# joesound212985/Deepfake-Detection-using-CLIP-Based-SigLIP-2-Vision-Transformers

Hardware: AMD Instinct MI355X
Metric: images/sec (train fwd+bwd) SigLIP-2-so400m@384 bf16 (higher is better)
Workload: dtype bf16; 1 GPU; so400m-patch14-384 encoder+pool-head train fwd+bwd, 384x384, per-GPU batch 128, seeded random weights; global_batch=128, parallelism=dp1

## Files before the change

deepfake-detection-using-clip-based-siglip-2-vision-transformers_amd/csrc/attention.hip:

```cpp
#include <stdlib.h>

#include "attention.hip.h"

namespace sgl {

template <int DP>
struct AttnCfg {
  static constexpr int KS = DP / 16;
  static constexpr int DT = (DP + 31) / 32;
  static constexpr int CPR = DP / 8;
  static constexpr int RSTR = DP * 2 + 16;
  static constexpr int TSTR = 192;
  static constexpr int DSTR = 208;
  static constexpr int DIMG = (32 * (DSTR / 16) + 63) / 64 * 1024;
  static constexpr int RIMG = (32 * (RSTR / 16) + 63) / 64 * 1024;
  static constexpr int SMEM_FWD = 2 * (64 * RSTR + 64 * TSTR);
  static constexpr int SMEM_KV = 3 * (2 * DIMG + 32 * 8);
  static constexpr int SMEM_Q = 3 * (DIMG + RIMG);
};

__device__ __forceinline__ u32x4 a_ldg(__amdgpu_buffer_rsrc_t r, uint32_t off) {
  return __builtin_amdgcn_raw_buffer_load_b128(r, off, 0, 0);
}
template <typename T>
// ... 317 lines not shown
        for (int r = 0; r < 16; ++r) o[dt][r] *= alpha;
    }
    lo_x8<T> pb[4];
    pb[0] = pack8<T>(s0, 0);
    pb[1] = pack8<T>(s0, 8);
    pb[2] = pack8<T>(s1, 0);
    pb[3] = pack8<T>(s1, 8);
#pragma unroll
    for (int dt = 0; dt < C::DT; ++dt)
#pragma unroll
      for (int kk = 0; kk < 4; ++kk) o[dt] = MFMA32(lds_trfrag<T>(vb, C::TSTR, kk, dt * 32, lane), pb[kk], o[dt]);
  }
  const float l = l_run + __shfl_xor(l_run, 32, 64);
  const float inv = 1.0f / l;
  const int q = q0 + qi;
  if (q < N) {
    T* orow = out + (size_t)(sb.row0 + q) * ((size_t)H * dh) + hd * dh;
#pragma unroll
    for (int dt = 0; dt < C::DT; ++dt)
#pragma unroll
      for (int g4 = 0; g4 < 4; ++g4) {
        const int d = dt * 32 + 8 * g4 + 4 * hh;
        if (d < dh) {
          lo_x4<T> v4;
#pragma unroll
          for (int r = 0; r < 4; ++r) v4[r] = (T)(o[dt][4 * g4 + r] * inv);
          *reinterpret_cast<lo_x4<T>*>(orow + d) = v4;
        }
      }
    if (hh == 0) lse[(size_t)hd * Ttot + sb.row0 + q] = m_run * scale + __logf(l);
  }
}

template <typename T, int DP, bool TOK>
__global__ __launch_bounds__(256, 2) void attn_bwd_kv_kernel(const T* __restrict__ Q, const T* __restrict__ K,
                                                             const T* __restrict__ V, const T* __restrict__ dO,
                                                             const float* __restrict__ aux, T* __restrict__ dqkv,
                                                             int B, int H, int N, int dh, int ld, float c, float scale) {
  using C = AttnCfg<DP>;
  constexpr int QT = 32;
  constexpr int SC = C::DSTR / 16;
  constexpr int NIS = (QT * SC + 63) / 64;
  constexpr int IMG = NIS * 1024;
  constexpr int STAGE = 2 * IMG + QT * 8;
  constexpr int NSLOT = 2 * NIS + 1;
  static_assert(NSLOT <= 16 && NSLOT > 12, "four DMA slots per wave (three for the last wave)");
  extern __shared__ __attribute__((aligned(16))) char smem[];
  const int t = threadIdx.x, lane = t & 63;
  const int w = __builtin_amdgcn_readfirstlane(t >> 6);
  int bh, xb;
  if (!head_block((N + 127) / 128, B * H, bh, xb)) return;
  const int b = bh / H, hd = bh - b * H;
  const int D = H * dh;
  const int key0 = xb * 128 + w * 32;
  HeadSrc src = head_src(TOK ? ld : 0, b, hd, H, N, dh, DP);
  if constexpr (!TOK) {
    src.rowbytes = (uint32_t)DP * 2u;
    src.nc = (uint32_t)DP / 8u;
  }
  const __amdgpu_buffer_rsrc_t rk = make_rsrc(K + src.base, src.bytes);
  const __amdgpu_buffer_rsrc_t rv = make_rsrc(V + src.base, src.bytes);
  const T* dOb = dO + (size_t)b * N * D + hd * dh;
  const u32x4 dq_ = att_desc(Q + src.base, src.bytes);
  const u32x4 ddo = att_desc(dOb, (uint32_t)(((size_t)(N - 1) * D + dh) * 2));
  const u32x4 dax = att_desc(aux + (size_t)bh * N * 2, (uint32_t)((size_t)N * 8));
  const uint32_t lds0 = (uint32_t)(size_t)((SGL_LDS char*)smem);
// ... 324 lines not shown
#pragma unroll
          for (int r = 0; r < 4; ++r) a[r] = (T)dq[dt][4 * g4 + r];
          *reinterpret_cast<lo_x4<T>*>(qrow + d) = a;
        }
      }
  }
}

bool attn_shape_ok(int dtype, int B, int H, int N, int dh, int DP, int ld, AttnPass pass) {
  const bool probs = pass == ATTN_PROBS, strict = dtype == DT_F32, f32m = dtype == DT_F32_MFMA;
  const bool lo = !strict && !f32m;
  if (probs && (B < 1 || H < 1 || N < 1 || dh < 1 || dh > DP)) return false;
  if (strict) {
    if (dh > 128) return false;
  } else {
    if (dh % 8) return false;
    if (f32m && (dh > 96 || DP < dh || DP % 4)) return false;
    if (lo && (DP != ((dh + 15) / 16) * 16 || !attn_dp_ok(DP))) return false;
    if (ld < 0 || (ld > 0 && (ld % (lo ? 8 : 4) || ld < H * dh))) return false;
  }
  if (f32m && N <= 0) return false;
  if (lo) {
    if ((size_t)N * (ld > 0 ? ld : DP) * 2 >= (1ull << 31)) return false;
    if (!probs && (size_t)N * H * dh * 2 >= (1ull << 31)) return false;
  }
  if (strict && !probs && attn_ref_lds(N, pass == ATTN_BWD ? 2 : 1, pass == ATTN_BWD ? 2 : 1) > 160 * 1024) return false;
  if (probs) {
    const size_t wgs = strict ? (size_t)((N + 3) / 4) * ((N + 63) / 64) : (size_t)((N + 127) / 128) * ((N + 127) / 128);
    if (wgs * (size_t)B * (size_t)H >= (1ull << 31)) return false;
  }
  return true;
}

hipError_t attn_fwd(const void* q, const void* k, const void* v, int dtype, void* out, float* lse, int B, int H, int N,
                    int dh, int DP, int ld, hipStream_t s) {
  if (B * H == 0 || N == 0) return hipSuccess;
  if (!attn_shape_ok(dtype, B, H, N, dh, DP, ld, ATTN_FWD)) return hipErrorInvalidValue;
  if (dtype == DT_F32)
    return attn_ref_fwd((const float*)q, (const float*)k, (const float*)v, (float*)out, lse, B, H, N, dh, DP, ld, s);
  if (dtype == DT_F32_MFMA)
    return attn_f32_fwd((const float*)q, (const float*)k, (const float*)v, (float*)out, lse, B, H, N, dh, DP, ld, s);
  if (!attn_aligned16(q, k, v)) return hipErrorInvalidValue;
  const AttnScales sc = attn_scales(dh);
  return dispatch_attn(dtype, DP, [&](auto tag) {
    using T = typename decltype(tag)::type;
    constexpr int DPV = decltype(tag)::dp;
    return with_bool(ld > 0, [&](auto tok) {
      hipLaunchKernelGGL((attn_fwd_kernel<T, DPV, tok.value>), head_grid((N + 127) / 128, B * H), dim3(256),
                         AttnCfg<DPV>::SMEM_FWD, s, (const T*)q, (const T*)k, (const T*)v, (T*)out, lse, B, H, N, dh,
                         tok.value ? ld : 0, sc.c, sc.scale);
      return hipGetLastError();
    });
  });
}

bool attn_varlen_shape_ok(int dtype, int S, int T, int max_n, int H, int dh, int DP) {
  if (S < 1 || T < 1 || max_n < 1 || H < 1 || dh < 1 || dh > DP) return false;
  if (!attn_shape_ok(dtype, 1, H, max_n, dh, DP, 0, ATTN_FWD)) return false;
  const int rows = dtype == DT_F32 ? 4 : 128;
  return seg_grid_ok(S, H, (max_n + rows - 1) / rows);
}

hipError_t attn_fwd_varlen(const void* q, const void* k, const void* v, int dtype, void* out, float* lse, const int* cu,
                           int S, int T, int max_n, int H, int dh, int DP, hipStream_t s) {
  if (!attn_varlen_shape_ok(dtype, S, T, max_n, H, dh, DP)) return hipErrorInvalidValue;
  if (dtype == DT_F32)
    return attn_ref_fwd_varlen((const float*)q, (const float*)k, (const float*)v, (float*)out, lse, cu, S, T, max_n, H, dh,
                               DP, s);
  if (dtype == DT_F32_MFMA)
    return attn_f32_fwd_varlen((const float*)q, (const float*)k, (const float*)v, (float*)out, lse, cu, S, T, max_n, H, dh,
                               DP, s);
  if (!attn_aligned16(q, k, v)) return hipErrorInvalidValue;
  const AttnScales sc = attn_scales(dh);
  return dispatch_attn(dtype, DP, [&](auto tag) {
    using T16 = typename decltype(tag)::type;
    constexpr int DPV = decltype(tag)::dp;
    hipLaunchKernelGGL((attn_fwd_varlen_kernel<T16, DPV>), seg_grid((max_n + 127) / 128, S * H), dim3(256),
                       AttnCfg<DPV>::SMEM_FWD, s, (const T16*)q, (const T16*)k, (const T16*)v, (T16*)out, lse, cu, S, T,
                       max_n, H, dh, sc.c, sc.scale);
// ... 36 lines not shown
```

deepfake-detection-using-clip-based-siglip-2-vision-transformers_amd/csrc/attention.hip.h:

```cpp
#pragma once
#include <math.h>

#include <type_traits>

#include "common.hip.h"
#include "kernels.h"

namespace sgl {

constexpr float kLog2e = SGL_LOG2E;
struct AttnScales {
  float scale, c;
};
static inline AttnScales attn_scales(int dh) {
  const float scale = 1.0f / sqrtf((float)dh);
  return {scale, scale * kLog2e};
}

__host__ __device__ constexpr int ctile_row(int i, int hh) { return 8 * (i >> 2) + 4 * hh + (i & 3); }

struct HeadSrc {
  uint32_t rowbytes, nc, bytes;
  size_t base;
};
// ... 27 lines not shown
  row0 = lo;
  n = min(hi - lo, max_n);
}
__device__ __forceinline__ bool seg_block(const int* __restrict__ cu, int S, int T, int max_n, int H, int nb, int rows,
                                          SegBlock& sb) {
  const int pid = blockIdx.x, xcd = pid & 7, slot = pid >> 3;
  const int hq = slot / nb;
  const int sh = hq * 8 + xcd;
  if (sh >= S * H) return false;
  sb.xb = slot - hq * nb;
  sb.seg = sh / H;
  sb.hd = sh - sb.seg * H;
  seg_range(cu, sb.seg, T, max_n, sb.row0, sb.n);
  return sb.xb * rows < sb.n;
}
static inline dim3 seg_grid(int nb, int SH) { return dim3((unsigned)(8 * ((SH + 7) / 8) * nb)); }
static inline bool seg_grid_ok(int S, int H, int nb) { return (size_t)8 * (((size_t)S * H + 7) / 8) * (size_t)nb < (1ull << 31); }

constexpr int kAttnDP[] = {16, 32, 48, 64, 80, 96};
constexpr int kAttnNDP = sizeof(kAttnDP) / sizeof(kAttnDP[0]);
constexpr bool attn_dp_ok(int DP) {
  for (int i = 0; i < kAttnNDP; ++i)
    if (kAttnDP[i] == DP) return true;
  return false;
}
constexpr size_t attn_ref_lds(int N, int nvec, int nrow) { return (size_t)4 * (nvec * N + 128 * nrow) * sizeof(float); }

enum AttnPass : int { ATTN_FWD, ATTN_BWD, ATTN_PROBS };
bool attn_shape_ok(int dtype, int B, int H, int N, int dh, int DP, int ld, AttnPass pass);
static inline bool attn_aligned16(const void* a, const void* b, const void* c = nullptr) {
  return ((((uintptr_t)a) | ((uintptr_t)b) | ((uintptr_t)c)) & 15) == 0;
}

template <typename T, int DP>
struct AttnTag {
  using type = T;
  static constexpr int dp = DP;
};
template <typename T, int I = 0, typename F>
hipError_t dispatch_attn_dp(int DP, F&& f) {
  if constexpr (I == kAttnNDP) {
    return hipErrorInvalidValue;
  } else {
    if (DP == kAttnDP[I]) return f(AttnTag<T, kAttnDP[I]>{});
    return dispatch_attn_dp<T, I + 1>(DP, f);
  }
}
template <typename F>
hipError_t dispatch_attn(int dtype, int DP, F&& f) {
  return dtype == DT_F16 ? dispatch_attn_dp<f16>(DP, f) : dispatch_attn_dp<bf16>(DP, f);
}
template <typename F>
auto with_bool(bool flag, F&& f) {
  return flag ? f(std::true_type{}) : f(std::false_type{});
}

hipError_t attn_f32_fwd(const float* q, const float* k, const float* v, float* out, float* lse, int B, int H, int N, int dh,
                        int DP, int ld, hipStream_t s);
hipError_t attn_f32_bwd(const float* q, const float* k, const float* v, const float* out, const float* dout,
                        const float* lse, float* dqkv, float* delta, int B, int H, int N, int dh, int DP, int ld,
                        hipStream_t s);
hipError_t attn_ref_fwd(const float* q, const float* k, const float* v, float* out, float* lse, int B, int H, int N, int dh,
                        int DP, int ld, hipStream_t s);
hipError_t attn_ref_bwd(const float* q, const float* k, const float* v, const float* out, const float* dout,
                        const float* lse, float* dqkv, float* delta, int B, int H, int N, int dh, int DP, int ld,
                        hipStream_t s);
// ... 7 lines not shown
```

deepfake-detection-using-clip-based-siglip-2-vision-transformers_amd/csrc/encoder.hip:

```cpp
#include <hip/hip_runtime.h>
#include <string.h>

#include <algorithm>
#include <new>
#include <vector>

#include "kernels.h"
#include "siglip_hip.h"

using namespace sgl;

namespace {

inline size_t align256(size_t x) { return (x + 255) & ~(size_t)255; }
inline char* at(void* base, size_t off) { return reinterpret_cast<char*>(base) + off; }
inline const char* at(const void* base, size_t off) { return reinterpret_cast<const char*>(base) + off; }
inline bool mfma16(int dt) { return dt == DT_BF16 || dt == DT_F16; }
inline int round_up(int x, int m) { return (x + m - 1) / m * m; }

struct Bump {
  size_t off = 0;
  size_t take(size_t bytes) {
    const size_t o = off;
    off += align256(bytes);
// ... 1378 lines not shown
  else if (dtype == DT_F16)
    CKV(gemm_nt_f16(A, lda, B, ldb, M, N, K, epi, out_dt, p, (hipStream_t)stream));
  else
    CKV(gemm_f32_generic((const float*)A, lda, 1, (const float*)B, ldb, 1, M, N, K, epi, out_dt, p,
                         (hipStream_t)stream));
  return SGL_OK;
}

int sgl_op_gemm_tn(int dtype, const void* A, int lda, const void* B, int ldb, int Mred, int N1, int N2, int splits,
                   float* out, int ldo, int accumulate, sgl_stream stream) {
  return sgl_op_gemm_tn_ws(dtype, A, lda, B, ldb, Mred, N1, N2, splits, out, ldo, accumulate, nullptr, 0, stream);
}

int sgl_op_gemm_tn_ws(int dtype, const void* A, int lda, const void* B, int ldb, int Mred, int N1, int N2, int splits,
                      float* out, int ldo, int accumulate, float* scratch, size_t scratch_bytes, sgl_stream stream) {
  EpiParams p;
  p.out = out; p.ldo = ldo; p.accumulate = accumulate;
  if (dtype == DT_BF16)
    CKV(gemm_tn_bf16(A, lda, B, ldb, Mred, N1, N2, splits, p, (hipStream_t)stream, scratch, scratch_bytes));
  else if (dtype == DT_F16)
    CKV(gemm_tn_f16(A, lda, B, ldb, Mred, N1, N2, splits, p, (hipStream_t)stream, scratch, scratch_bytes));
  else
    CKV(gemm_f32_generic((const float*)A, 1, lda, (const float*)B, 1, ldb, N1, N2, Mred, EPI_F32, DT_F32, p,
                         (hipStream_t)stream));
  return SGL_OK;
}

int sgl_op_attn_fwd(int dtype, const void* q, const void* k, const void* v, void* out, float* lse, int B, int H, int N,
                    int head_dim, int head_dim_pad, int ld_qkv, sgl_stream stream) {
  CKV(attn_fwd(q, k, v, dtype, out, lse, B, H, N, head_dim, head_dim_pad, ld_qkv, (hipStream_t)stream));
  return SGL_OK;
}

int sgl_op_attn_bwd(int dtype, const void* q, const void* k, const void* v, const void* out, const void* dout,
                    const float* lse, void* dqkv, float* delta_scratch, int B, int H, int N, int head_dim,
                    int head_dim_pad, int ld_qkv, sgl_stream stream) {
  CKV(attn_bwd(q, k, v, out, dout, lse, dtype, dqkv, delta_scratch, B, H, N, head_dim, head_dim_pad, ld_qkv, (hipStream_t)stream));
  return SGL_OK;
}

int sgl_op_attn_probs(int dtype, const void* q, const void* k, const float* lse, float* out, int B, int H, int N,
                      int head_dim, int head_dim_pad, int mode, sgl_stream stream) {
  if (!q || !k || !lse || !out) return SGL_ERR_NULL;
  if (B < 1 || H < 1 || N < 1 || head_dim < 1 || head_dim_pad < 1 || head_dim > head_dim_pad) return SGL_ERR_BAD_SHAPE;
  if (dtype != DT_F32 && dtype != DT_BF16 && dtype != DT_F32_MFMA && dtype != DT_F16) return SGL_ERR_UNSUPPORTED;
  if (mode != SGL_ATTN_PROBS_FULL && mode != SGL_ATTN_PROBS_HEAD_MEAN) return SGL_ERR_UNSUPPORTED;
  if (!attn_probs_shape_ok(dtype, B, H, N, head_dim, head_dim_pad)) return SGL_ERR_BAD_SHAPE;
  CKV(attn_probs(q, k, lse, out, dtype, B, H, N, head_dim, head_dim_pad, mode, (hipStream_t)stream));
  return SGL_OK;
}

int sgl_op_attn_grad_probs(int dtype, const void* q, const void* k, const void* v, const void* dout, const float* lse,
                           float* out, int B, int H, int N, int head_dim, int head_dim_pad, int kind, int mode,
                           sgl_stream stream) {
  if (!q || !k || !v || !dout || !lse || !out) return SGL_ERR_NULL;
  if (B < 1 || H < 1 || N < 1 || head_dim < 1 || head_dim_pad < 1 || head_dim > head_dim_pad) return SGL_ERR_BAD_SHAPE;
  if (dtype != DT_F32 && dtype != DT_BF16 && dtype != DT_F32_MFMA && dtype != DT_F16) return SGL_ERR_UNSUPPORTED;
  if (mode != SGL_ATTN_PROBS_FULL && mode != SGL_ATTN_PROBS_HEAD_MEAN) return SGL_ERR_UNSUPPORTED;
  if (kind != SGL_ATTN_GRAD_DP && kind != SGL_ATTN_GRAD_PDP && kind != SGL_ATTN_GRAD_RELEVANCE) return SGL_ERR_UNSUPPORTED;
  if (!attn_grad_probs_shape_ok(dtype, B, H, N, head_dim, head_dim_pad)) return SGL_ERR_BAD_SHAPE;
  CKV(attn_grad_probs(q, k, v, dout, lse, out, dtype, B, H, N, head_dim, head_dim_pad, kind, mode, (hipStream_t)stream));
  return SGL_OK;
}

int sgl_attention_probs(sgl_ctx* ctx, int B, int H, int W, const void* saved, size_t saved_bytes, int layer, int mode,
                        float* out, size_t out_bytes, sgl_stream stream) {
// ... 233 lines not shown
```

deepfake-detection-using-clip-based-siglip-2-vision-transformers_amd/csrc/kernels.h:

```cpp
#pragma once
#include <hip/hip_runtime.h>
#include <stddef.h>
#include <stdint.h>

#include "siglip_hip.h"

namespace sgl {

enum DType : int {
  DT_F32 = 0,
  DT_BF16 = 1,
  DT_F32_MFMA = 2,
  DT_F16 = 3,
};
static inline size_t dtype_size(int dt) { return (dt == DT_BF16 || dt == DT_F16) ? 2 : 4; }

template <auto Kernel>
hipError_t set_max_dynamic_lds_once(int bytes) {
  static bool done = false;
  if (done) return hipSuccess;
  const hipError_t e =
      hipFuncSetAttribute(reinterpret_cast<const void*>(Kernel), hipFuncAttributeMaxDynamicSharedMemorySize, bytes);
  done = e == hipSuccess;
  return e;
// ... 142 lines not shown
constexpr TnPlan tn_plan(int Mred, int N1, int N2, size_t ws_bytes, int tile = 0) {
  TnPlan best = {0, 0, 0};
  long best_cost = 0;
  for (int g = 0; g < 2; ++g) {
    const int bm = g ? 384 : 256, bn = g ? 192 : 256, area8 = g ? 9 : 8;
    if (tile != 0 && tile != bm) continue;
    const int tiles = ((N1 + bm - 1) / bm) * ((N2 + bn - 1) / bn);
    for (int sp = 1; sp == 1 || (tiles * sp <= 256 && Mred / sp >= 1024); ++sp) {
      if (sp > 1 && (size_t)sp * N1 * N2 * sizeof(float) > ws_bytes) break;
      const int m_per = ((Mred + sp - 1) / sp + 63) / 64 * 64;
      const long cost = (long)area8 * m_per;
      if (best.tile == 0 || cost < best_cost) {
        best = {bm, (Mred + m_per - 1) / m_per, m_per};
        best_cost = cost;
      }
    }
  }
  return best;
}
constexpr bool tn_plan_is(int Mred, int N1, int N2, size_t ws_bytes, int tile, int splits) {
  const TnPlan p = tn_plan(Mred, N1, N2, ws_bytes);
  return (tile == 0 || p.tile == tile) && p.splits == splits;
}
constexpr size_t kTnSlabBytes = (size_t)256 * 384 * 192 * 4;
static_assert(tn_plan_is(93312, 1152, 1152, kTnSlabBytes, 384, 14), "out_proj dW");
static_assert(tn_plan_is(93312, 3456, 1152, kTnSlabBytes, 384, 4), "QKV dW");
static_assert(tn_plan_is(93312, 4304, 1152, kTnSlabBytes, 256, 3), "fc1 dW");
static_assert(tn_plan_is(93312, 1152, 4304, kTnSlabBytes, 256, 3), "fc2 dW");
static_assert(tn_plan_is(4133, 520, 1152, kTnSlabBytes, 0, 4) && tn_plan(4133, 520, 1152, kTnSlabBytes).m_per == 1088, "digest case");
static_assert(tn_plan_is(2048, 512, 512, kTnSlabBytes, 256, 2) && tn_plan(2048, 512, 512, kTnSlabBytes).m_per == 1024, "digest case");

hipError_t attn_fwd(const void* q, const void* k, const void* v, int dtype, void* out, float* lse, int B, int H,
                    int N, int dh, int DP, int ld_qkv, hipStream_t s);
bool attn_varlen_shape_ok(int dtype, int S, int T, int max_n, int H, int dh, int DP);
hipError_t attn_fwd_varlen(const void* q, const void* k, const void* v, int dtype, void* out, float* lse, const int* cu,
                           int S, int T, int max_n, int H, int dh, int DP, hipStream_t s);
hipError_t attn_bwd(const void* q, const void* k, const void* v, const void* out, const void* dout,
                    const float* lse, int dtype, void* dqkv, float* delta, int B, int H, int N, int dh, int DP,
                    int ld_qkv, hipStream_t s);

bool attn_probs_shape_ok(int dtype, int B, int H, int N, int dh, int DP);
hipError_t attn_probs(const void* q, const void* k, const float* lse, float* out, int dtype, int B, int H, int N, int dh,
                      int DP, int mode, hipStream_t s);
hipError_t probs_head_mean(const float* probs, float* out, int B, int H, int N, hipStream_t s);

bool attn_grad_probs_shape_ok(int dtype, int B, int H, int N, int dh, int DP);
hipError_t attn_grad_probs(const void* q, const void* k, const void* v, const void* dout, const float* lse, float* out,
                           int dtype, int B, int H, int N, int dh, int DP, int kind, int mode, hipStream_t s);
hipError_t pool_attn_grad_probs(const void* V, int dtype, const float* probs, const float* dout ,
                                float* out, int B, int H, int N, int dh, int DP, int kind, int mode, hipStream_t s);

}
```

deepfake-detection-using-clip-based-siglip-2-vision-transformers_amd/lib.py:

```python
from __future__ import annotations

import ctypes as C
import os
import re

_HERE = os.path.dirname(os.path.abspath(__file__))
LIB_PATH = os.environ.get("SGL_LIB_PATH") or os.path.join(_HERE, "libsiglip_hip.so")
HEADER_PATH = os.path.join(os.path.dirname(_HERE), "include", "siglip_hip.h")

SGL_DTYPE_F32, SGL_DTYPE_BF16, SGL_DTYPE_BF16X3, SGL_DTYPE_F16, SGL_DTYPE_MXFP8 = 0, 1, 2, 3, 5
SGL_DTYPE_U8 = 6
SEG_EVAL_AUC_BINS = 4096
SEG_TERM_FOCAL, SEG_TERM_BOUNDARY, SEG_TERM_TV = 1, 2, 4
SGL_RECOMPUTE_NONE, SGL_RECOMPUTE_BLOCKS = 0, 1
ATTN_PROBS_FULL, ATTN_PROBS_HEAD_MEAN = 0, 1
ATTN_GRAD_DP, ATTN_GRAD_PDP, ATTN_GRAD_RELEVANCE = 0, 1, 2
EPI_STORE, EPI_BIAS_GELU, EPI_RES_F32, EPI_QKV, EPI_GELU_BWD, EPI_POS_F32, EPI_F32 = range(7)
STATUS = {0: "ok", -1: "bad shape", -2: "unsupported configuration", -3: "buffer too small", -4: "HIP error",
          -5: "null pointer"}

_fp = C.c_void_p


class SglConfig(C.Structure):
# ... 105 lines not shown
    _sig(lib, "sgl_query_sizes_ragged", i, [C.c_void_p, C.POINTER(C.c_int), i, psz])
    _sig(lib, "sgl_forward_ragged", i, [C.c_void_p, C.POINTER(SglWeights), _fp, _fp, C.POINTER(C.c_int), i, C.POINTER(_fp),
                                        _fp, _fp, _fp, sz, _fp])
    _sig(lib, "sgl_backward_begin_p", i, [C.c_void_p, C.POINTER(SglWeights), _fp, C.POINTER(SglGrads), i, i, i, _fp, _fp,
                                          _fp, _fp, _fp, sz, _fp, sz, _fp])
    _sig(lib, "sgl_backward_layer_p", i, [C.c_void_p, C.POINTER(SglWeights), _fp, C.POINTER(SglGrads), i, i, i, i, _fp,
                                          _fp, i, _fp, sz, _fp, sz, _fp])
    preq = C.POINTER(SglAttnGradReq)
    _sig(lib, "sgl_backward_begin_pa", i, [C.c_void_p, C.POINTER(SglWeights), _fp, C.POINTER(SglGrads), i, i, i, _fp, _fp,
                                           _fp, _fp, _fp, sz, _fp, sz, _fp, preq])
    _sig(lib, "sgl_backward_layer_pa", i, [C.c_void_p, C.POINTER(SglWeights), _fp, C.POINTER(SglGrads), i, i, i, i, _fp,
                                           _fp, i, _fp, sz, _fp, sz, _fp, preq])
    _sig(lib, "sgl_backward_begin", i, [C.c_void_p, C.POINTER(SglWeights), _fp, C.POINTER(SglGrads), i, i, i, _fp, _fp,
                                        _fp, _fp, _fp, sz, _fp, sz, _fp])
    _sig(lib, "sgl_backward_layer", i, [C.c_void_p, C.POINTER(SglWeights), _fp, C.POINTER(SglGrads), i, i, i, i, _fp,
                                        _fp, i, _fp, sz, _fp, sz, _fp])
    _sig(lib, "sgl_backward_embed", i, [C.c_void_p, C.POINTER(SglWeights), C.POINTER(SglGrads), i, i, i, i, _fp, sz,
                                        _fp, sz, _fp])
    _sig(lib, "sgl_query_input_grad_bytes", i, [C.c_void_p, i, i, i, psz])
    _sig(lib, "sgl_backward_embed_px", i, [C.c_void_p, C.POINTER(SglWeights), C.POINTER(SglGrads), i, i, i, i, _fp, i, _fp,
                                           sz, _fp, sz, _fp, sz, _fp])
    _sig(lib, "sgl_backward", i, [C.c_void_p, C.POINTER(SglWeights), _fp, C.POINTER(SglGrads), i, i, i, i, _fp,
                                  C.POINTER(_fp), _fp, _fp, i, i, _fp, sz, _fp, sz, _fp])
    _sig(lib, "sgl_op_layernorm_fwd", i, [_fp, _fp, _fp, _fp, i, _fp, _fp, i, i, f, _fp])
    _sig(lib, "sgl_op_layernorm_bwd", i, [_fp, i, _fp, _fp, _fp, _fp, _fp, _fp, _fp, i, _fp, _fp, _fp, sz, i, i, _fp])
    _sig(lib, "sgl_op_gemm_nt", i, [i, _fp, i, _fp, i, i, i, i, i, _fp, i, _fp, i, _fp, _fp, i, _fp, i, _fp, i, i, i,
                                    i, i, i, _fp])
    _sig(lib, "sgl_op_quantize_mxfp8", i, [_fp, i, i, i, i, i, _fp, _fp, _fp])
    _sig(lib, "sgl_op_layernorm_fwd_mx", i, [_fp, _fp, _fp, _fp, _fp, i, i, i, f, _fp])
    _sig(lib, "sgl_op_gemm_nt_mx", i, [_fp, _fp, _fp, _fp, i, i, i, i, _fp, i, _fp, _fp, _fp, i, i, i, i, i, i, _fp])
    _sig(lib, "sgl_op_gemm_tn", i, [i, _fp, i, _fp, i, i, i, i, i, _fp, i, i, _fp])
    _sig(lib, "sgl_op_gemm_tn_ws", i, [i, _fp, i, _fp, i, i, i, i, i, _fp, i, i, _fp, sz, _fp])
    _sig(lib, "sgl_op_attn_fwd", i, [i, _fp, _fp, _fp, _fp, _fp, i, i, i, i, i, i, _fp])
    _sig(lib, "sgl_op_attn_bwd", i, [i, _fp, _fp, _fp, _fp, _fp, _fp, _fp, _fp, i, i, i, i, i, i, _fp])
    _sig(lib, "sgl_op_attn_probs", i, [i, _fp, _fp, _fp, _fp, i, i, i, i, i, i, _fp])
    _sig(lib, "sgl_op_attn_grad_probs", i, [i, _fp, _fp, _fp, _fp, _fp, _fp, i, i, i, i, i, i, i, _fp])
    _sig(lib, "sgl_op_pool_attn_grad_probs", i, [i, _fp, _fp, _fp, _fp, i, i, i, i, i, i, i, _fp])
    _sig(lib, "sgl_attention_probs", i, [C.c_void_p, i, i, i, _fp, sz, i, i, _fp, sz, _fp])
    _sig(lib, "sgl_op_colsum", i, [i, _fp, i, i, i, _fp, i, _fp, sz, _fp])
    _sig(lib, "sgl_op_im2col", i, [_fp, i, _fp, i, i, i, i, i, i, _fp])
    _sig(lib, "sgl_op_col2im", i, [_fp, i, i, i, i, i, _fp, i, _fp])
    _sig(lib, "sgl_op_pos_resize", i, [_fp, i, _fp, i, i, i, _fp])
    _sig(lib, "sgl_op_pool_attn_fwd", i, [i, _fp, _fp, _fp, _fp, _fp, i, i, i, i, i, _fp])
    _sig(lib, "sgl_op_attn_fwd_varlen", i, [i, _fp, _fp, _fp, _fp, _fp, _fp, i, i, i, i, i, i, _fp])
    _sig(lib, "sgl_op_pool_attn_fwd_varlen", i, [i, _fp, _fp, _fp, _fp, _fp, _fp, i, i, i, i, i, i, _fp])
    _sig(lib, "sgl_op_seg_offsets", i, [C.POINTER(C.c_int), i, _fp, _fp])
    _sig(lib, "sgl_op_pool_attn_bwd", i, [i, _fp, _fp, _fp, _fp, _fp, _fp, _fp, i, i, i, i, i, _fp])
    _sig(lib, "sgl_op_pos_resize_bwd", i, [_fp, i, i, _fp, i, i, _fp])
    _sig(lib, "sgl_op_cast_pad", i, [_fp, i, i, i, _fp, i, i, i, i, _fp])
    _sig(lib, "sgl_op_cast_job", i, [C.POINTER(SglCastMat), i, C.POINTER(SglCastVec), i, i, _fp])
    _sig(lib, "sgl_op_split3", i, [_fp, i, i, i, _fp, i, i, i, _fp])
    _sig(lib, "sgl_op_batch_sum", i, [_fp, i, sz, _fp, i, _fp])
    _sig(lib, "sgl_op_vecmat", i, [_fp, _fp, i, i, _fp, sz, _fp, i, _fp])
    _sig(lib, "sgl_op_reduce_partials", i, [_fp, i, i, _fp, i, i, _fp])
    _sig(lib, "sgl_op_reduce_partials3", i, [_fp, i, i, _fp, _fp, _fp, i, i, i, i, _fp])
    _sig(lib, "sgl_op_reduce_splits", i, [_fp, i, sz, i, i, _fp, i, i, _fp])
    _sig(lib, "sgl_op_add_f32", i, [_fp, _fp, _fp, sz, _fp])
    _sig(lib, "sgl_op_cast_f32", i, [_fp, _fp, i, sz, _fp])
    i64 = C.c_int64
    _sig(lib, "sgl_adamw_plan", i64, [C.POINTER(C.c_uint64), i, C.POINTER(C.c_int32), i64])
    _sig(lib, "sgl_op_grad_norm", i, [_fp, _fp, i64, f, _fp, _fp, _fp])
    _sig(lib, "sgl_op_adamw", i, [_fp, _fp, i64, C.c_double, C.c_double, C.c_double, i, _fp, _fp])
    _sig(lib, "sgl_op_ema", i, [_fp, _fp, i64, C.c_double, _fp])
    _sig(lib, "sgl_adamw_bind_shadows", i, [C.c_void_p, C.POINTER(SglWeights), _fp, C.POINTER(SglAdamwTensor),
                                            C.POINTER(SglAdamwAux), i])
    _sig(lib, "sgl_op_grad_norm_scaled", i, [_fp, _fp, i64, f, f, _fp, _fp, _fp])
# ... 73 lines not shown
```

include/siglip_hip.h:

```cpp
#ifndef SIGLIP_HIP_H
#define SIGLIP_HIP_H
#include <stddef.h>
#include <stdint.h>

#ifdef __cplusplus
extern "C" {
#endif

typedef struct sgl_ctx sgl_ctx;
typedef void* sgl_stream;

enum { SGL_DTYPE_F32 = 0, SGL_DTYPE_BF16 = 1, SGL_DTYPE_BF16X3 = 2, SGL_DTYPE_F16 = 3, SGL_DTYPE_MXFP8 = 5 };
enum { SGL_DTYPE_U8 = 6 };

typedef enum {
  SGL_OK = 0,
  SGL_ERR_BAD_SHAPE = -1,
  SGL_ERR_UNSUPPORTED = -2,
  SGL_ERR_WORKSPACE = -3,
  SGL_ERR_HIP = -4,
  SGL_ERR_NULL = -5
} sgl_status;

typedef struct {
// ... 96 lines not shown
int sgl_backward_embed_px(sgl_ctx* ctx, const sgl_weights* w, const sgl_grads* g, int B, int H, int W,
                          int interpolate_pos, float* d_pixels, int channels_last, void* px_scratch,
                          size_t px_scratch_bytes, const void* saved, size_t saved_bytes, void* ws, size_t ws_bytes,
                          sgl_stream stream);
int sgl_backward(sgl_ctx* ctx, const sgl_weights* w, const void* shadow, const sgl_grads* g, int B, int H, int W,
                 int interpolate_pos, const float* hidden_states, const float* const* d_taps,
                 const float* d_last_hidden, const float* d_pooled, int first_trainable_block, int train_embeddings,
                 const void* saved, size_t saved_bytes, void* ws, size_t ws_bytes, sgl_stream stream);

int sgl_op_layernorm_fwd(const float* x, const float* gamma, const float* beta, void* y, int y_dtype, float* mean,
                         float* rstd, int M, int D, float eps, sgl_stream stream);
int sgl_op_layernorm_bwd(const void* dy, int dy_dtype, const float* x, const float* mean, const float* rstd,
                         const float* gamma, const float* dres, float* dx, void* dx_lp, int lp_dtype, float* dgamma,
                         float* dbeta, float* scratch, size_t scratch_bytes, int M, int D, sgl_stream stream);
enum { SGL_EPI_STORE = 0, SGL_EPI_BIAS_GELU = 1, SGL_EPI_RES_F32 = 2, SGL_EPI_QKV = 3, SGL_EPI_GELU_BWD = 4,
       SGL_EPI_POS_F32 = 5, SGL_EPI_F32 = 6 };
int sgl_op_gemm_nt(int dtype, const void* A, int lda, const void* B, int ldb, int M, int N, int K, int epi, void* out,
                   int ldo, void* out2, int ldo2, const float* bias, const float* res, int ldr, const void* aux,
                   int ldaux, const float* pos, int pos_rows, int tokens, int heads, int head_dim, int head_dim_pad,
                   int batch, sgl_stream stream);
int sgl_op_quantize_mxfp8(const void* x, int x_dtype, int ldx, int M, int K, int Kp, void* q, void* scales,
                          sgl_stream stream);
int sgl_op_layernorm_fwd_mx(const float* x, const float* gamma, const float* beta, void* q, void* scales, int M, int D,
                            int Kp, float eps, sgl_stream stream);
int sgl_op_gemm_nt_mx(const void* A, const void* As, const void* B, const void* Bs, int M, int N, int Kp, int epi,
                      void* out, int ldo, void* out_scales, const float* bias, const float* res, int ldr, int tokens,
                      int heads, int head_dim, int head_dim_pad, int batch, sgl_stream stream);
int sgl_op_gemm_tn(int dtype, const void* A, int lda, const void* B, int ldb, int Mred, int N1, int N2, int splits,
                   float* out, int ldo, int accumulate, sgl_stream stream);
int sgl_op_gemm_tn_ws(int dtype, const void* A, int lda, const void* B, int ldb, int Mred, int N1, int N2, int splits,
                      float* out, int ldo, int accumulate, float* scratch, size_t scratch_bytes, sgl_stream stream);
int sgl_op_attn_fwd(int dtype, const void* q, const void* k, const void* v, void* out, float* lse, int B, int H, int N,
                    int head_dim, int head_dim_pad, int ld_qkv, sgl_stream stream);
int sgl_op_attn_bwd(int dtype, const void* q, const void* k, const void* v, const void* out, const void* dout,
                    const float* lse, void* dqkv, float* delta_scratch, int B, int H, int N, int head_dim,
                    int head_dim_pad, int ld_qkv, sgl_stream stream);
enum { SGL_ATTN_PROBS_FULL = 0, SGL_ATTN_PROBS_HEAD_MEAN = 1 };
int sgl_op_attn_probs(int dtype, const void* q, const void* k, const float* lse, float* out, int B, int H, int N,
                      int head_dim, int head_dim_pad, int mode, sgl_stream stream);
int sgl_attention_probs(sgl_ctx* ctx, int B, int H, int W, const void* saved, size_t saved_bytes, int layer, int mode,
                        float* out, size_t out_bytes, sgl_stream stream);
enum { SGL_ATTN_GRAD_DP = 0, SGL_ATTN_GRAD_PDP = 1, SGL_ATTN_GRAD_RELEVANCE = 2 };
int sgl_op_attn_grad_probs(int dtype, const void* q, const void* k, const void* v, const void* dout, const float* lse,
                           float* out, int B, int H, int N, int head_dim, int head_dim_pad, int kind, int mode,
                           sgl_stream stream);
int sgl_op_pool_attn_grad_probs(int dtype, const void* V, const float* probs, const float* dout, float* out, int B, int H,
                                int N, int head_dim, int head_dim_pad, int kind, int mode, sgl_stream stream);
typedef struct {
  float* out;
  size_t out_bytes;
  int kind;
  int mode;
} sgl_attn_grad_req;
int sgl_backward_layer_pa(sgl_ctx* ctx, const sgl_weights* w, const void* shadow, const sgl_grads* g, int layer, int B,
                          int H, int W, const float* hs_in, const float* d_tap, int need_dx, const void* saved,
                          size_t saved_bytes, void* ws, size_t ws_bytes, sgl_stream stream,
                          const sgl_attn_grad_req* req);
int sgl_backward_begin_pa(sgl_ctx* ctx, const sgl_weights* w, const void* shadow, const sgl_grads* g, int B, int H, int W,
                          const float* hs_last, const float* d_last_hidden, const float* d_pooled,
                          const float* d_tap_last, const void* saved, size_t saved_bytes, void* ws, size_t ws_bytes,
                          sgl_stream stream, const sgl_attn_grad_req* req);
int sgl_op_colsum(int dtype, const void* in, int ld, int M, int N, float* out, int accumulate, float* scratch,
                  size_t scratch_bytes, sgl_stream stream);
int sgl_op_im2col(const float* pixels, int channels_last, void* out, int out_dtype, int B, int H, int W, int P, int Kp,
                  sgl_stream stream);
int sgl_op_col2im(const float* d_cols, int B, int H, int W, int P, int Kp, float* d_pixels, int channels_last,
// ... 162 lines not shown
```

Before: 447.3 images/sec.

## Add 64-row-per-wave attention forward kernel reusing K/V fragments across query blocks

```diff
diff --git a/deepfake-detection-using-clip-based-siglip-2-vision-transformers_amd/csrc/attention.hip b/deepfake-detection-using-clip-based-siglip-2-vision-transformers_amd/csrc/attention.hip
--- a/deepfake-detection-using-clip-based-siglip-2-vision-transformers_amd/csrc/attention.hip
+++ b/deepfake-detection-using-clip-based-siglip-2-vision-transformers_amd/csrc/attention.hip
@@ -373,6 +373,175 @@
   }
 }
 
+template <typename T, int DP>
+__global__ __launch_bounds__(256, 2) void attn_fwd64_kernel(const T* __restrict__ Q, const T* __restrict__ K,
+                                                            const T* __restrict__ V, T* __restrict__ out,
+                                                            float* __restrict__ lse, int B, int H, int N, int dh, float c,
+                                                            float scale) {
+  using C = AttnCfg<DP>;
+  constexpr int KT = 64, NB = 2;
+  constexpr int KBYTES = KT * C::RSTR, VBYTES = KT * C::TSTR, STAGE = KBYTES + VBYTES;
+  constexpr int SCK = C::RSTR / 16, SCV = C::TSTR / 16;
+  constexpr int NIK = KT * SCK / 64, NIV = KT * SCV / 64, NSLOT = NIK + NIV;
+  constexpr int NPW = (NSLOT + 3) / 4;
+  extern __shared__ __attribute__((aligned(16))) char smem[];
+  const int t = threadIdx.x, lane = t & 63;
+  const int w = __builtin_amdgcn_readfirstlane(t >> 6);
+  int bh, xb;
+  if (!head_block((N + 255) / 256, B * H, bh, xb)) return;
+  const int b = bh / H, hd = bh - b * H;
+  const int q0 = xb * 256 + w * 64;
+  HeadSrc src = head_src(0, b, hd, H, N, dh, DP);
+  src.rowbytes = (uint32_t)DP * 2u;
+  src.nc = (uint32_t)DP / 8u;
+  const __amdgpu_buffer_rsrc_t rq = make_rsrc(Q + src.base, src.bytes);
+  const u32x4 dk_ = att_desc(K + src.base, src.bytes);
+  const u32x4 dv_ = att_desc(V + src.base, src.bytes);
+  const uint32_t lds0 = (uint32_t)(size_t)((SGL_LDS char*)smem);
+
+  const int qi = lane & 31, hh = lane >> 5;
+  lo_x8<T> qf[NB][C::KS];
+#pragma unroll
+  for (int blk = 0; blk < NB; ++blk)
+#pragma unroll
+    for (int ks = 0; ks < C::KS; ++ks) {
+      const uint32_t ch = (uint32_t)(2 * ks + hh);
+      const int qr = q0 + 32 * blk + qi;
+      qf[blk][ks] = as_x8<T>(a_ldg(rq, (qr < N && ch < src.nc) ? (uint32_t)qr * src.rowbytes + ch * 16u : SGL_OOB));
+    }
+
+  uint32_t voff[NPW];
+#pragma unroll
+  for (int j = 0; j < NPW; ++j) {
+    const int sl = w + 4 * j;
+    voff[j] = (sl < NIK) ? att_chunk_off(sl * 64 + lane, KT, SCK, (int)src.nc, src.rowbytes)
+                         : att_chunk_off((sl - NIK) * 64 + lane, KT, SCV, (int)src.nc, src.rowbytes);
+  }
+  const uint32_t tile_adv = (uint32_t)KT * src.rowbytes;
+  auto issue = [&](int stage) {
+    const uint32_t sb = lds0 + (uint32_t)(stage * STAGE);
+#pragma unroll
+    for (int j = 0; j < NPW; ++j) {
+      const int sl = w + 4 * j;
+      if (sl < NSLOT) att_dma16(sl < NIK ? dk_ : dv_, sb + (uint32_t)sl * 1024u, voff[j]);
+      voff[j] += tile_adv;
+    }
+  };
+
+  float m_run[NB], l_run[NB];
+  f32x16 o[NB][C::DT];
+#pragma unroll
+  for (int blk = 0; blk < NB; ++blk) {
+    m_run[blk] = -INFINITY;
+    l_run[blk] = 0.f;
+#pragma unroll
+    for (int dt = 0; dt < C::DT; ++dt)
+#pragma unroll
+      for (int r = 0; r < 16; ++r) o[blk][dt][r] = 0.f;
+  }
+
+  const int ntiles = (N + KT - 1) / KT;
+#pragma unroll
+  for (int blk = 0; blk < NB; ++blk)
+#pragma unroll
+    for (int ks = 0; ks < C::KS; ++ks) asm volatile("" ::"v"(qf[blk][ks]));
+  asm volatile("s_waitcnt vmcnt(0)" ::: "memory");
+  issue(0);
+  for (int tile = 0; tile < ntiles; ++tile) {
+    const int cur = tile & 1;
+    SGL_ATT_WAIT_BARRIER(0);
+    if (tile + 1 < ntiles) issue(cur ^ 1);
+    const char* kb = smem + cur * STAGE;
+    const char* vb = kb + KBYTES;
+    f32x16 s0[NB], s1[NB];
+#pragma unroll
+    for (int blk = 0; blk < NB; ++blk)
+#pragma unroll
+      for (int r = 0; r < 16; ++r) { s0[blk][r] = 0.f; s1[blk][r] = 0.f; }
+#pragma unroll
+    for (int ks = 0; ks < C::KS; ++ks) {
+      const lo_x8<T> k0 = lds_row8<T>(kb + qi * C::RSTR + (16 * ks + 8 * hh) * 2);
+      const lo_x8<T> k1 = lds_row8<T>(kb + (qi + 32) * C::RSTR + (16 * ks + 8 * hh) * 2);
+#pragma unroll
+      for (int blk = 0; blk < NB; ++blk) {
+        s0[blk] = MFMA32(k0, qf[blk][ks], s0[blk]);
+        s1[blk] = MFMA32(k1, qf[blk][ks], s1[blk]);
+      }
+    }
+    lo_x8<T> pb[NB][4];
+#pragma unroll
+    for (int blk = 0; blk < NB; ++blk) {
+      if (tile == ntiles - 1) {
+#pragma unroll
+        for (int r = 0; r < 16; ++r) {
+          const int key = tile * KT + (r & 3) + 8 * (r >> 2) + 4 * hh;
+          if (key >= N) s0[blk][r] = -INFINITY;
+          if (key + 32 >= N) s1[blk][r] = -INFINITY;
+        }
+      }
+      float mx = s0[blk][0];
+#pragma unroll
+      for (int r = 1; r < 16; ++r) mx = fmaxf(mx, s0[blk][r]);
+#pragma unroll
+      for (int r = 0; r < 16; ++r) mx = fmaxf(mx, s1[blk][r]);
+      mx = fmaxf(mx, __shfl_xor(mx, 32, 64));
+      const float m_new = fmaxf(m_run[blk], mx);
+      const bool grew = __any(m_new > m_run[blk]);
+      const float alpha = grew ? fast_exp2(c * (m_run[blk] - m_new)) : 1.0f;
+      const float mc = m_new * c;
+      float rs = 0.f;
+#pragma unroll
+      for (int r = 0; r < 16; ++r) {
+        s0[blk][r] = fast_exp2(fmaf(s0[blk][r], c, -mc));
+        s1[blk][r] = fast_exp2(fmaf(s1[blk][r], c, -mc));
+        rs += s0[blk][r] + s1[blk][r];
+      }
+      l_run[blk] = l_run[blk] * alpha + rs;
+      m_run[blk] = m_new;
+      if (grew) {
+#pragma unroll
+        for (int dt = 0; dt < C::DT; ++dt)
+#pragma unroll
+          for (int r = 0; r < 16; ++r) o[blk][dt][r] *= alpha;
+      }
+      pb[blk][0] = pack8<T>(s0[blk], 0);
+      pb[blk][1] = pack8<T>(s0[blk], 8);
+      pb[blk][2] = pack8<T>(s1[blk], 0);
+      pb[blk][3] = pack8<T>(s1[blk], 8);
+    }
+#pragma unroll
+    for (int dt = 0; dt < C::DT; ++dt)
+#pragma unroll
+      for (int kk = 0; kk < 4; ++kk) {
+        const lo_x8<T> vf = lds_trfrag<T>(vb, C::TSTR, kk, dt * 32, lane);
+#pragma unroll
+        for (int blk = 0; blk < NB; ++blk) o[blk][dt] = MFMA32(vf, pb[blk][kk], o[blk][dt]);
+      }
+  }
+#pragma unroll
+  for (int blk = 0; blk < NB; ++blk) {
+    const float l = l_run[blk] + __shfl_xor(l_run[blk], 32, 64);
+    const float inv = 1.0f / l;
+    const int q = q0 + 32 * blk + qi;
+    if (q < N) {
+      T* orow = out + ((size_t)b * N + q) * ((size_t)H * dh) + hd * dh;
+#pragma unroll
+      for (int dt = 0; dt < C::DT; ++dt)
+#pragma unroll
+        for (int g4 = 0; g4 < 4; ++g4) {
+          const int d = dt * 32 + 8 * g4 + 4 * hh;
+          if (d < dh) {
+            lo_x4<T> v4;
+#pragma unroll
+            for (int r = 0; r < 4; ++r) v4[r] = (T)(o[blk][dt][4 * g4 + r] * inv);
+            *reinterpret_cast<lo_x4<T>*>(orow + d) = v4;
+          }
+        }
+      if (hh == 0) lse[(size_t)bh * N + q] = m_run[blk] * scale + __logf(l);
+    }
+  }
+}
+
 template <typename T, int DP, bool TOK>
 __global__ __launch_bounds__(256, 2) void attn_bwd_kv_kernel(const T* __restrict__ Q, const T* __restrict__ K,
                                                              const T* __restrict__ V, const T* __restrict__ dO,
@@ -763,6 +932,11 @@
   return true;
 }
 
+int attn_fwd_form(int dtype, int DP, int ld, int N, int forced) {
+  static const int rows_env = getenv("SGL_ATTN_FWD_ROWS") ? atoi(getenv("SGL_ATTN_FWD_ROWS")) : 0;
+  return attn_fwd_rows(dtype, DP, ld, N, forced < 0 ? rows_env : forced);
+}
+
 hipError_t attn_fwd(const void* q, const void* k, const void* v, int dtype, void* out, float* lse, int B, int H, int N,
                     int dh, int DP, int ld, hipStream_t s) {
   if (B * H == 0 || N == 0) return hipSuccess;
@@ -773,9 +947,18 @@
     return attn_f32_fwd((const float*)q, (const float*)k, (const float*)v, (float*)out, lse, B, H, N, dh, DP, ld, s);
   if (!attn_aligned16(q, k, v)) return hipErrorInvalidValue;
   const AttnScales sc = attn_scales(dh);
+  const int rows = attn_fwd_form(dtype, DP, ld, N, -1);
   return dispatch_attn(dtype, DP, [&](auto tag) {
     using T = typename decltype(tag)::type;
     constexpr int DPV = decltype(tag)::dp;
+    if constexpr (attn_fwd64_dp_ok(DPV)) {
+      if (rows == 64) {
+        hipLaunchKernelGGL((attn_fwd64_kernel<T, DPV>), head_grid((N + 255) / 256, B * H), dim3(256),
+                           AttnCfg<DPV>::SMEM_FWD, s, (const T*)q, (const T*)k, (const T*)v, (T*)out, lse, B, H, N, dh, sc.c,
+                           sc.scale);
+        return hipGetLastError();
+      }
+    }
     return with_bool(ld > 0, [&](auto tok) {
       hipLaunchKernelGGL((attn_fwd_kernel<T, DPV, tok.value>), head_grid((N + 127) / 128, B * H), dim3(256),
                          AttnCfg<DPV>::SMEM_FWD, s, (const T*)q, (const T*)k, (const T*)v, (T*)out, lse, B, H, N, dh,
diff --git a/deepfake-detection-using-clip-based-siglip-2-vision-transformers_amd/csrc/attention.hip.h b/deepfake-detection-using-clip-based-siglip-2-vision-transformers_amd/csrc/attention.hip.h
--- a/deepfake-detection-using-clip-based-siglip-2-vision-transformers_amd/csrc/attention.hip.h
+++ b/deepfake-detection-using-clip-based-siglip-2-vision-transformers_amd/csrc/attention.hip.h
@@ -83,6 +83,20 @@
   return ((((uintptr_t)a) | ((uintptr_t)b) | ((uintptr_t)c)) & 15) == 0;
 }
 
+constexpr int kAttnFwd64DP[] = {64, 80};
+constexpr bool attn_fwd64_dp_ok(int DP) {
+  for (int v : kAttnFwd64DP)
+    if (v == DP) return true;
+  return false;
+}
+constexpr int kAttnFwd64MinN = 196;
+constexpr int attn_fwd_rows(int dtype, int DP, int ld, int N, int forced) {
+  const bool legal64 = dtype != DT_F32 && dtype != DT_F32_MFMA && ld == 0 && attn_fwd64_dp_ok(DP);
+  if (!legal64 || forced == 32) return 32;
+  if (forced == 64) return 64;
+  return N >= kAttnFwd64MinN ? 64 : 32;
+}
+
 template <typename T, int DP>
 struct AttnTag {
   using type = T;
diff --git a/deepfake-detection-using-clip-based-siglip-2-vision-transformers_amd/csrc/encoder.hip b/deepfake-detection-using-clip-based-siglip-2-vision-transformers_amd/csrc/encoder.hip
--- a/deepfake-detection-using-clip-based-siglip-2-vision-transformers_amd/csrc/encoder.hip
+++ b/deepfake-detection-using-clip-based-siglip-2-vision-transformers_amd/csrc/encoder.hip
@@ -1434,6 +1434,10 @@
   return SGL_OK;
 }
 
+int sgl_op_attn_fwd_rows(int dtype, int head_dim_pad, int ld_qkv, int N, int forced) {
+  return attn_fwd_form(dtype, head_dim_pad, ld_qkv, N, forced);
+}
+
 int sgl_op_attn_bwd(int dtype, const void* q, const void* k, const void* v, const void* out, const void* dout,
                     const float* lse, void* dqkv, float* delta_scratch, int B, int H, int N, int head_dim,
                     int head_dim_pad, int ld_qkv, sgl_stream stream) {
diff --git a/deepfake-detection-using-clip-based-siglip-2-vision-transformers_amd/csrc/kernels.h b/deepfake-detection-using-clip-based-siglip-2-vision-transformers_amd/csrc/kernels.h
--- a/deepfake-detection-using-clip-based-siglip-2-vision-transformers_amd/csrc/kernels.h
+++ b/deepfake-detection-using-clip-based-siglip-2-vision-transformers_amd/csrc/kernels.h
@@ -198,6 +198,7 @@
 
 hipError_t attn_fwd(const void* q, const void* k, const void* v, int dtype, void* out, float* lse, int B, int H,
                     int N, int dh, int DP, int ld_qkv, hipStream_t s);
+int attn_fwd_form(int dtype, int DP, int ld_qkv, int N, int forced);
 bool attn_varlen_shape_ok(int dtype, int S, int T, int max_n, int H, int dh, int DP);
 hipError_t attn_fwd_varlen(const void* q, const void* k, const void* v, int dtype, void* out, float* lse, const int* cu,
                            int S, int T, int max_n, int H, int dh, int DP, hipStream_t s);
diff --git a/deepfake-detection-using-clip-based-siglip-2-vision-transformers_amd/lib.py b/deepfake-detection-using-clip-based-siglip-2-vision-transformers_amd/lib.py
--- a/deepfake-detection-using-clip-based-siglip-2-vision-transformers_amd/lib.py
+++ b/deepfake-detection-using-clip-based-siglip-2-vision-transformers_amd/lib.py
@@ -161,6 +161,7 @@
     _sig(lib, "sgl_op_gemm_tn", i, [i, _fp, i, _fp, i, i, i, i, i, _fp, i, i, _fp])
     _sig(lib, "sgl_op_gemm_tn_ws", i, [i, _fp, i, _fp, i, i, i, i, i, _fp, i, i, _fp, sz, _fp])
     _sig(lib, "sgl_op_attn_fwd", i, [i, _fp, _fp, _fp, _fp, _fp, i, i, i, i, i, i, _fp])
+    _sig(lib, "sgl_op_attn_fwd_rows", i, [i, i, i, i, i])
     _sig(lib, "sgl_op_attn_bwd", i, [i, _fp, _fp, _fp, _fp, _fp, _fp, _fp, _fp, i, i, i, i, i, i, _fp])
     _sig(lib, "sgl_op_attn_probs", i, [i, _fp, _fp, _fp, _fp, i, i, i, i, i, i, _fp])
     _sig(lib, "sgl_op_attn_grad_probs", i, [i, _fp, _fp, _fp, _fp, _fp, _fp, i, i, i, i, i, i, i, _fp])
diff --git a/include/siglip_hip.h b/include/siglip_hip.h
--- a/include/siglip_hip.h
+++ b/include/siglip_hip.h
@@ -152,6 +152,7 @@
                       float* out, int ldo, int accumulate, float* scratch, size_t scratch_bytes, sgl_stream stream);
 int sgl_op_attn_fwd(int dtype, const void* q, const void* k, const void* v, void* out, float* lse, int B, int H, int N,
                     int head_dim, int head_dim_pad, int ld_qkv, sgl_stream stream);
+int sgl_op_attn_fwd_rows(int dtype, int head_dim_pad, int ld_qkv, int N, int forced);
 int sgl_op_attn_bwd(int dtype, const void* q, const void* k, const void* v, const void* out, const void* dout,
                     const float* lse, void* dqkv, float* delta_scratch, int B, int H, int N, int head_dim,
                     int head_dim_pad, int ld_qkv, sgl_stream stream);
```

Measured after the change: 447.8 images/sec, median of 6. Within noise of the previous version (+0.1%).
